# youmi-zym/GO-SLAM

Hardware: AMD Instinct MI355X
Metric: BA keyframes/s (6 x FactorGraph.update: reproject + corr lookup + GRU + 2 GN BA iters) on synthetic 640x480 RGB-D (higher is better)
Workload: dtype f32 (BA/geometry; fp64 solve), f16 (corr volume, GRU convs); 1 GPU; configs[1]-shaped frontend window: 60x80 maps (480x640 RGB-D), P=25 keyframes, E=75 edges, 6 updates/keyframe, iters=2, RGB-D depth prior, upsample on; parallelism=replicas x1 (tracking does not shard)

## Files before the change

go_slam_amd/_lib.py:

```python
import ctypes
import os
import subprocess

_HERE = os.path.dirname(os.path.abspath(__file__))
CSRC = os.path.join(_HERE, "csrc")
LIB_PATH = os.environ.get("GOSLAM_HIP_LIB") or os.path.join(CSRC, "libgoslam_hip.so")

_lib = None

c_int, c_float, c_void_p, c_size_t = ctypes.c_int, ctypes.c_float, ctypes.c_void_p, ctypes.c_size_t

_P = c_void_p
SIGNATURES = {
    "gs_version": (ctypes.c_char_p, []),
    "gs_last_error": (ctypes.c_char_p, []),
    "gs_enc_conv_wpack_elems": (c_size_t, [c_int, c_int, c_int]),
    "gs_enc_conv_stat_chunks": (c_int, [c_int, c_int, c_int]),
    "gs_enc_conv": (c_int, [_P, c_int, c_int, _P, _P, _P, c_int, c_int, c_int, c_int, c_int, c_int, c_int, _P, _P, _P]),
    "gs_norm_act_workspace_bytes_chunks": (c_size_t, [c_int, c_int, c_int]),
    "gs_timing_begin": (c_int, [_P]),
    "gs_timing_end": (c_int, []),
    "gs_timing_read": (c_int, [ctypes.c_char_p, ctypes.POINTER(ctypes.c_double), ctypes.POINTER(c_int)]),
    "gs_timing_names": (c_int, [ctypes.c_char_p, c_int]),
    "gs_corr_index_forward": (c_int, [_P, _P, _P] + [c_int] * 7 + [_P]),
# ... 11 lines not shown
    "gs_altcorr_pyramid": (c_int, [_P] * 8 + [c_int] * 5 + [_P]),
    "gs_reproject": (c_int, [_P] * 7 + [c_int] * 3 + [_P]),
    "gs_projmap": (c_int, [_P] * 7 + [c_int] * 3 + [_P]),
    "gs_frame_distance": (c_int, [_P] * 6 + [c_int] * 3 + [c_float, _P]),
    "gs_iproj": (c_int, [_P] * 4 + [c_int] * 3 + [_P]),
    "gs_depth_filter": (c_int, [_P] * 6 + [c_int] * 4 + [_P]),
    "gs_pointcloud_workspace_bytes": (c_size_t, [c_int] * 3),
    "gs_pointcloud_count": (c_int, [_P] * 5 + [c_float, c_float] + [c_int] * 4 + [_P, c_size_t, _P]),
    "gs_pointcloud_mask": (c_int, [_P, _P] + [c_int] * 4 + [_P, c_size_t, _P]),
    "gs_pointcloud_scan": (c_int, [c_int] * 3 + [_P, c_size_t, _P, _P]),
    "gs_pointcloud_emit": (c_int, [_P] * 5 + [c_int] * 4 + [_P, c_size_t, ctypes.c_longlong, _P, _P, _P]),
    "gs_tsdf_batch": (c_int, []),
    "gs_tsdf_integrate": (c_int, [_P] * 3 + [c_int] * 3 + [_P] * 4 + [c_int] * 3 + [c_float] * 10 + [_P]),
    "gs_tsdf_vertex_attr": (c_int, [_P, c_int, _P, _P, c_int, c_int, c_int, c_float, _P, _P, _P]),
    "gs_frame_prep_color": (c_int, [_P, c_int, c_int, c_int, c_int, c_int, _P]),
    "gs_frame_prep_depth": (c_int, [_P, c_int, c_float, c_int, c_int, c_int, c_int, _P]),
    "gs_cvx_upsample":(c_int, [_P] * 4 + [c_int] * 4 + [_P]),
    "gs_upmask_upsample": (c_int, [_P, c_int, _P, _P, _P, _P, _P, c_int, c_int, c_int, _P]),
    "gs_bias_act": (c_int, [_P, _P, _P, c_int, c_int, c_int, c_int, c_int, _P]),
    "gs_motion_features": (c_int, [_P, _P, _P, c_int, c_int, c_int, _P]),
    "gs_ba_inputs": (c_int, [_P] * 6 + [c_int, c_int, c_int, _P]),
    "gs_lowmem_gather": (c_int, [_P] * 7 + [c_int, c_int, c_int, _P]),
    "gs_lowmem_scatter": (c_int, [_P] * 8 + [c_int, c_int, c_int, _P]),
    "gs_damping_rows": (c_int, [_P] * 5 + [c_int, c_int, c_float, c_float, _P]),
    "gs_conv1x1": (c_int, [_P, c_int, c_int, _P, _P, c_int, _P, c_int, c_int, ctypes.c_longlong, _P]),
    "gs_conv7x7_c4": (c_int, [_P, _P, _P, _P, c_int, c_int, c_int, c_int, c_int, c_int, _P]),
    "gs_conv3x3_wpack_elems": (c_size_t, [c_int, c_int]),
    "gs_conv3x3_pp": (c_int, [_P, c_int, c_int, _P, c_int, _P, c_int, c_int, c_int, c_int, c_int, c_int, _P]),
    "gs_conv3x3_bias_relu": (c_int, [_P, c_int, c_int, _P, _P, _P, c_int, c_int, c_int, c_int, c_int, _P]),
    "gs_conv3x3_gru_zr": (c_int, [_P, c_int, c_int, _P, _P, _P, _P, _P, _P, c_int, c_int, c_int, _P]),
    "gs_conv3x3_gru_zr2": (c_int, [_P, _P, c_int, c_int, _P, _P, _P, _P, _P, _P, c_int, c_int, c_int, _P]),
    "gs_conv3x3_gru_q": (c_int, [_P, _P, c_int, c_int, _P, _P, _P, _P, _P, _P, _P, c_int, c_int, c_int, _P]),
    "gs_conv3x3_head": (c_int, [_P, c_int, _P, c_int, _P, _P, c_int, c_int, c_float, _P, c_int, c_int, c_int, _P]),
    "gs_segment_mean": (c_int, [_P, c_int, _P, c_int, _P, _P, _P, c_int, c_int, c_int, _P]),
    "gs_norm_act_workspace_bytes": (c_size_t, [c_int, c_int, c_int]),
    "gs_norm_act": (c_int, [_P, _P, _P, _P] + [c_int] * 6 + [c_float, _P, c_size_t, c_int, _P]),
    "gs_gru_glo_workspace_bytes": (c_size_t, [c_int]),
    "gs_gru_glo": (c_int, [_P] * 11 + [c_int, c_int, _P, c_size_t, _P]),
    "gs_gru_glo_fused_workspace_bytes": (c_size_t, [c_int, c_int]),
    "gs_gru_glo_fused": (c_int, [_P, c_int] + [_P] * 10 + [c_int, c_int, _P, c_size_t, _P]),
    "gs_gru_gate_zr": (c_int, [_P] * 6 + [c_int] * 3 + [_P]),
    "gs_gru_gate_q": (c_int, [_P] * 7 + [c_int] * 2 + [_P]),
    "gs_edge_prep": (c_int, [_P] * 4 + [c_int, _P, _P] + [c_int] * 6 + [c_float, c_int, c_int, _P]),
    "gs_edge_greedy": (c_int, [_P] * 5 + [c_int] * 5 + [c_float, c_int, c_int, _P]),
    "gs_ba_workspace_bytes": (c_size_t, [c_int] * 5),
    "gs_ba": (c_int, [_P] * 9 + [c_int] * 3 + [c_float, c_float] + [c_int] * 6 + [_P, _P, _P, _P, c_size_t, _P]),
    "gs_ba_ex": (c_int, [_P] * 9 + [c_int] * 3 + [c_float, c_float] + [c_int] * 6 + [_P, _P, _P, _P, c_size_t, c_int, _P]),
    "gs_chol_solve": (c_int, [_P, _P, c_int, c_float, c_float, c_int, _P, _P, _P]),
    "gs_traj_eval_workspace_bytes": (c_size_t, [c_int]),
    "gs_traj_world": (c_int, [_P, _P, c_int, _P, _P, _P]),
    "gs_ape_moments": (c_int, [_P, _P, _P, c_int, _P, _P, c_size_t, _P]),
    "gs_ape_stats": (c_int, [_P, _P, _P, _P, c_int, _P, _P, _P, c_size_t, _P]),
    "gs_grid_meta_default": (c_int, [_P]),
    "gs_neus_level_major_min_points": (c_int, [c_int]),
    "gs_render_sample": (c_int, [_P] * 7 + [c_float, _P, _P, _P] + [c_int] * 3 + [_P]),
    "gs_grid_encode": (c_int, [_P] * 4 + [c_int, _P]),
    "gs_grid_backward": (c_int, [_P, _P, _P, c_int, c_float, _P, _P, c_int, c_float, _P, _P, c_int, _P]),
    "gs_mlp_workspace_bytes": (c_size_t, [c_int, c_int]),
    "gs_mlp_forward": (c_int, [_P] * 3 + [c_int] * 3 + [_P, c_size_t, _P]),
    "gs_neus_forward_workspace_bytes": (c_size_t, [c_int, c_int]),
    "gs_neus_forward": (c_int, [_P] * 9 + [c_float] + [_P] * 18 + [c_float, _P, c_float, c_int, c_int, _P, c_size_t, _P]),
    "gs_neus_forward_pieces": (c_int, [c_int] * 3),
    "gs_neus_forward_segmented": (c_int, [_P] * 9 + [c_float] + [_P] * 18 + [c_float, c_int, _P, _P, c_float]
                                  + [c_int] * 4 + [_P, c_size_t, _P]),
    "gs_render_img_sample": (c_int, [_P, c_int, c_int] + [c_float] * 4 + [_P] * 5 + [c_int] + [_P] * 5
                             + [c_int, c_int, _P]),
# ... 155 lines not shown
```

go_slam_amd/csrc/conv3x3_pp.hip:

```cpp
#include "common.h"
#include "conv3x3_common.h"

namespace {

constexpr int PP_KG = 4;
constexpr int PP_PSTR = 5;
constexpr int pp_zpad(int tw) { return (((2 * (tw + 2) + 2) * PP_PSTR + 3 + 15) / 16) * 16; }
constexpr int pp_patch_slots(int tw) {
  return (((512 / tw + 2) * (tw + 2) * PP_PSTR + 511) / 512) * 512 + pp_zpad(tw);
}

__device__ __attribute__((aligned(16))) const uint32_t pp_zero_page[4] = {0u, 0u, 0u, 0u};

__device__ __forceinline__ void pp_glds16(const void* src, void* lds_wave_base) {
  __builtin_amdgcn_global_load_lds((const __attribute__((address_space(1))) void*)src,
                                   (__attribute__((address_space(3))) void*)lds_wave_base, 16, 0, 0);
}

#define PP_BAR()                              \
  do {                                        \
    asm volatile("" ::: "memory");            \
    __builtin_amdgcn_s_barrier();             \
    asm volatile("" ::: "memory");            \
    __builtin_amdgcn_sched_barrier(0);        \
  } while (0)

#define PP_LGKM0()                                        \
  do {                                                    \
    asm volatile("s_waitcnt lgkmcnt(0)" ::: "memory");    \
    __builtin_amdgcn_sched_barrier(0);                    \
  } while (0)

struct PpEpi {
  const float* bias;
  const float* glo;
  const _Float16* inp_pre;
  const _Float16* aux0;
  const _Float16* aux1;
  _Float16* out0;
  _Float16* out1;
  const _Float16* xb;
  int xsb, split;
  long long* dbg;
  int variant;
};

template <bool PROBE>
__device__ __forceinline__ void pp_stamp(long long* dbg, int slot) {
  if constexpr (PROBE) {
    if (dbg && threadIdx.x == 0) dbg[(size_t)blockIdx.x * 4 + slot] = (long long)__builtin_amdgcn_s_memtime();
  }
}

__device__ __forceinline__ float pp_sigm(float v) { return gs_sigmoid(v); }

template <int TW, int EPI, int BN = 128, bool PROBE = false>
__global__ __launch_bounds__(512, 1) void conv3x3_pp_kernel(const _Float16* __restrict__ x, int xs, int C,
                                                            const half8* __restrict__ wpack, _Float16* __restrict__ y,
                                                            int ys, int H, int W, int rows, int tiles_x, int NB,
                                                            int xcd, PpEpi ep) {
  static_assert(BN == 128 || (BN == 64 && (EPI == 0 || EPI == 3)), "64-channel workgroups: plain / bias + ReLU only");
  constexpr int PP_BN = BN;
  constexpr int PP_WTAP = PP_KG * PP_BN;
  constexpr int NJ = BN / 64;
  constexpr int PP_TS = NJ == 2 ? 72 : 40;
  constexpr int TH_ = 512 / TW, PW_ = TW + 2, NPX = (TH_ + 2) * PW_;
  constexpr int PSTR = PP_PSTR;
  constexpr int ZPAD = pp_zpad(TW);
  constexpr int NROUND = (NPX * PSTR + 511) / 512;
  constexpr int PSLOTS = NROUND * 512 + ZPAD;
  constexpr int ZSLOT = NROUND * 512;
  static_assert(PSLOTS == pp_patch_slots(TW), "launch_pp sizes the LDS with the same formula");
  static_assert(NROUND <= 9, "one DMA round per tap");
  extern __shared__ half8 smem[];
  half8* const pbuf = smem;
// ... 144 lines not shown
  for (int ck = 0; ck < nchunk; ++ck) {
#pragma unroll
    for (int tap = 0; tap < 9; ++tap) {
      const int tg = ck * 9 + tap;
      __builtin_amdgcn_sched_barrier(0);
      math([&]() {
        if constexpr (PROBE) {
          if (ep.variant & 4) return;
        }
        const int tw = tg + 3 < T ? tg + 3 : T - 1;
        issue_w(tw, (tg + 3) & 3);
        if (tap < NROUND) issue_patch(ck + 1 < nchunk ? ck + 1 : nchunk - 1, (ck + 1) & 1, tap, poff[tap]);
      });
      __builtin_amdgcn_sched_barrier(0);
      if (tap < NROUND) asm volatile("s_waitcnt vmcnt(2)" ::: "memory");
      else asm volatile("s_waitcnt vmcnt(1)" ::: "memory");
      PP_BAR();
      bool reads = true;
      if constexpr (PROBE) reads = !(ep.variant & 8);
      if (reads) {
        if (tap < 8) read_frags(ck & 1, (tg + 1) & 3, tap + 1);
        else if (ck + 1 < nchunk) read_frags((ck + 1) & 1, (tg + 1) & 3, 0);
      }
      PP_LGKM0();
      PP_BAR();
    }
  }
  pp_stamp<PROBE>(ep.dbg, 2);
  if (grp2 == 0) PP_BAR();
  asm volatile("s_waitcnt vmcnt(0)" ::: "memory");
  PP_BAR();

  _Float16* tile = reinterpret_cast<_Float16*>(smem) + wv * 32 * PP_TS;
  _Float16* yb = y + nb * PP_BN + wn * (PP_BN / 2);
  constexpr int PIECES = NJ * 4;
  constexpr int PXIT = 64 / PIECES;
  constexpr int NIT = 32 / PXIT;
#pragma unroll
  for (int i = 0; i < 4; ++i) {
    size_t pix4[NIT];
    bool ok4[NIT];
    half8 pi4[NIT], u4[NIT], v4[NIT];
    const int piece = lane & (PIECES - 1);
    const int c8 = wn * (PP_BN / 2) + piece * 8;
#pragma unroll
    for (int it = 0; it < NIT; ++it) {
      const int pxr = it * PXIT + lane / PIECES;
      int ty, tx;
      tile_pixel<TW, true>(wm, i, pxr, ty, tx);
      const int gv = g0 + ty, gx = tx0 + tx;
      ok4[it] = gv < rows && gx < W;
      pix4[it] = (size_t)gv * W + gx;
      if constexpr (EPI == 1 || EPI == 2) {
        const half8 z8 = {0, 0, 0, 0, 0, 0, 0, 0};
        pi4[it] = z8; u4[it] = z8; v4[it] = z8;
        if (ok4[it]) {
          if constexpr (EPI == 1) {
            if (ep.inp_pre) pi4[it] = *reinterpret_cast<const half8*>(ep.inp_pre + pix4[it] * 384 + nb * 128 + c8);
            if (nb == 1) u4[it] = *reinterpret_cast<const half8*>(x + pix4[it] * xs + c8);
          } else {
            if (ep.inp_pre) pi4[it] = *reinterpret_cast<const half8*>(ep.inp_pre + pix4[it] * 384 + 256 + c8);
            u4[it] = *reinterpret_cast<const half8*>(ep.aux0 + pix4[it] * 128 + c8);
            v4[it] = *reinterpret_cast<const half8*>(ep.aux1 + pix4[it] * 128 + c8);
          }
        }
      }
    }
#pragma unroll
    for (int j = 0; j < NJ; ++j)
#pragma unroll
      for (int g = 0; g < 4; ++g) {
        half4 o;
#pragma unroll
        for (int e = 0; e < 4; ++e) o[e] = (_Float16)acc[j][i][4 * g + e];
        *reinterpret_cast<half4*>(tile + r * PP_TS + j * 32 + 8 * g + 4 * kgl) = o;
      }
    __builtin_amdgcn_fence(__ATOMIC_RELEASE, "wavefront");
    __builtin_amdgcn_wave_barrier();
    __builtin_amdgcn_fence(__ATOMIC_ACQUIRE, "wavefront");
#pragma unroll
    for (int it = 0; it < NIT; ++it) {
      const int pxr = it * PXIT + lane / PIECES;
      if (ok4[it]) {
        const half8 v = *reinterpret_cast<const half8*>(tile + pxr * PP_TS + piece * 8);
        const size_t pix = pix4[it];
        if constexpr (EPI == 0) {
          *reinterpret_cast<half8*>(yb + pix * ys + piece * 8) = v;
        } else if constexpr (EPI == 3) {
          const float* bb = ep.bias + nb * PP_BN + c8;
          half8 o;
#pragma unroll
          for (int k = 0; k < 8; ++k) o[k] = (_Float16)fmaxf((float)v[k] + bb[k], 0.0f);
          *reinterpret_cast<half8*>(yb + pix * ys + piece * 8) = o;
        } else if constexpr (EPI == 1) {
          const int img = (int)(pix / ((size_t)H * W));
          const half8 pi = pi4[it];
          const float* bb = ep.bias + nb * 128 + c8;
          const float* gg = ep.glo + (size_t)img * 256 + nb * 128 + c8;
          half8 o;
          if (nb == 0) {
#pragma unroll
            for (int k = 0; k < 8; ++k) o[k] = (_Float16)pp_sigm((float)v[k] + (float)pi[k] + bb[k] + gg[k]);
            *reinterpret_cast<half8*>(ep.out0 + pix * 128 + c8) = o;
          } else {
            const half8 net = u4[it];
#pragma unroll
            for (int k = 0; k < 8; ++k)
              o[k] = (_Float16)(pp_sigm((float)v[k] + (float)pi[k] + bb[k] + gg[k]) * (float)net[k]);
            *reinterpret_cast<half8*>(ep.out1 + pix * 128 + c8) = o;
          }
        } else {
          const int img = (int)(pix / ((size_t)H * W));
          const half8 pi = pi4[it], zz = u4[it], nn = v4[it];
          const float* bb = ep.bias + c8;
          const float* gg = ep.glo + (size_t)img * 128 + c8;
          half8 o;
#pragma unroll
          for (int k = 0; k < 8; ++k) {
            const float a_ = (float)v[k] + (float)pi[k] + bb[k] + gg[k];
// ... 113 lines not shown
  if (n == 0) return GS_OK;
  PpEpi ep = PpEpi();
  ep.bias = bias_q;
  ep.glo = glo_q;
  ep.inp_pre = (const _Float16*)inp_pre;
  ep.aux0 = (const _Float16*)z;
  ep.aux1 = (const _Float16*)net;
  ep.out0 = (_Float16*)net_out;
  ep.xb = (const _Float16*)x_rest;
  ep.xsb = x_rest_stride;
  ep.split = 128;
  return dispatch_pp<2>(rnet, 128, 128 + c_rest, wpack, pp_tile_width(w), nullptr, 0, 128, n, h, w, 1,
                        (hipStream_t)stream, ep);
}

extern "C" int gs_conv3x3_bias_relu(const void* x, int x_stride, int c_in, const void* wpack, const float* bias, void* y,
                                    int y_stride, int n_out, int n, int h, int w, gs_stream_t stream) {
  GS_REQUIRE(x && wpack && bias && y, "conv3x3_bias_relu: null pointer");
  GS_REQUIRE(c_in > 0 && c_in % 32 == 0, "conv3x3_bias_relu: c_in must be a multiple of 32");
  GS_REQUIRE(n_out > 0 && n_out % 64 == 0, "conv3x3_bias_relu: n_out must be a multiple of 64");
  GS_REQUIRE(x_stride >= c_in && x_stride % 8 == 0, "conv3x3_bias_relu: bad x_stride");
  GS_REQUIRE(y_stride >= n_out && y_stride % 8 == 0, "conv3x3_bias_relu: bad y_stride");
  GS_REQUIRE(n >= 0 && h > 0 && w > 0, "conv3x3_bias_relu: bad shape");
  if (n == 0) return GS_OK;
  PpEpi ep = PpEpi();
  ep.bias = bias;
  if (pp_block_channels(n_out) == 64)
    return dispatch_pp<3, 64>(x, x_stride, c_in, wpack, pp_tile_width(w), y, y_stride, n_out, n, h, w, 1,
                              (hipStream_t)stream, ep);
  return dispatch_pp<3>(x, x_stride, c_in, wpack, pp_tile_width(w), y, y_stride, n_out, n, h, w, 1, (hipStream_t)stream,
                        ep);
}

extern "C" size_t gs_conv3x3_wpack_elems(int c_in, int n_out) { return (size_t)9 * c_in * n_out; }

#ifdef GS_BUILD_PROBES
extern "C" int gs_conv3x3_pp_probe(const void* x, int x_stride, int c_in, const void* wpack, int tw, void* y, int y_stride,
                                   int n_out, int n, int h, int w, int variant, long long* dbg, gs_stream_t stream) {
  GS_REQUIRE(x && wpack && y, "conv3x3_pp_probe: null pointer");
  GS_REQUIRE(tw == 16 && c_in > 0 && c_in % 32 == 0 && n_out > 0 && n_out % 128 == 0 && n > 0,
             "conv3x3_pp_probe: bad arguments (tw must be 16)");
  PpEpi ep = PpEpi();
  ep.dbg = dbg;
  ep.variant = variant;
  return launch_pp<16, 0, 128, true>(x, x_stride, c_in, wpack, y, y_stride, n_out, n, h, w, 1, (hipStream_t)stream, ep);
}
#endif
```

go_slam_amd/csrc/conv_heads.hip:

```cpp
#include "common.h"

namespace {

typedef _Float16 half8 __attribute__((ext_vector_type(8)));
typedef float float16v __attribute__((ext_vector_type(16)));

constexpr int HEAD_ROWS = 6;

template <int O>
__global__ __launch_bounds__(256) void conv3x3_head_kernel(
    const _Float16* __restrict__ x, int ldx, const float* __restrict__ in_bias, int in_relu,
    const _Float16* __restrict__ wpack, const float* __restrict__ bias, int epilogue, float out_scale,
    float* __restrict__ out, int h, int w) {
  constexpr int NT = 9 * O;
  constexpr int S = NT | 1;
  extern __shared__ float cs[];
  const int n = blockIdx.y;
  const int r0 = blockIdx.x * HEAD_ROWS;
  const int in_lo = max(r0 - 1, 0), in_hi = min(r0 + HEAD_ROWS, h - 1);
  const int npx = (in_hi - in_lo + 1) * w;
  const int tid = threadIdx.x, lane = tid & 63, wv = tid >> 6;
  const int kh = 8 * (lane >> 5);

  half8 a[8];
// ... 57 lines not shown
  }
  __syncthreads();

  const int nrow = min(HEAD_ROWS, h - r0);
  for (int idx = tid; idx < nrow * w; idx += 256) {
    const int r = r0 + idx / w, cc = idx % w;
    float acc[O];
#pragma unroll
    for (int o = 0; o < O; ++o) acc[o] = 0.0f;
#pragma unroll
    for (int ky = 0; ky < 3; ++ky) {
      const int rr = r + ky - 1;
      if (rr < 0 || rr >= h) continue;
#pragma unroll
      for (int kx = 0; kx < 3; ++kx) {
        const int c2 = cc + kx - 1;
        if (c2 < 0 || c2 >= w) continue;
        const float* p = cs + ((rr - in_lo) * w + c2) * S + (ky * 3 + kx) * O;
#pragma unroll
        for (int o = 0; o < O; ++o) acc[o] += p[o];
      }
    }
    float* op = out + ((size_t)(n * h + r) * w + cc) * O;
#pragma unroll
    for (int o = 0; o < O; ++o) {
      float v = (float)(_Float16)(acc[o] + bias[o]);
      if (epilogue == 1) v = (float)(_Float16)gs_sigmoid(v);
      else if (epilogue == 2) v = (v > 20.0f) ? v : log1pf(__expf(v));
      op[o] = v * out_scale;
    }
  }
}

template <int O>
int launch_head(const void* x, int ldx, const float* in_bias, int in_relu, const void* wpack, const float* bias,
                int epilogue, float out_scale, float* out, int n, int h, int w, hipStream_t st) {
  constexpr int S = (9 * O) | 1;
  const size_t lds = (size_t)(HEAD_ROWS + 2) * w * S * sizeof(float);
  GS_REQUIRE(lds <= 160 * 1024 - 512, "conv3x3_head: image width %d needs %zu bytes of LDS", w, lds);
  static GsLdsLimit limit;
  if (int rc = limit.raise((const void*)conv3x3_head_kernel<O>, lds, "conv3x3_head")) return rc;
  conv3x3_head_kernel<O><<<dim3(gs_cdiv(h, HEAD_ROWS), n), 256, lds, st>>>(
      (const _Float16*)x, ldx, in_bias, in_relu, (const _Float16*)wpack, bias, epilogue, out_scale, out, h, w);
  GS_CHECK_LAUNCH("conv3x3_head");
  return GS_OK;
}

}

extern "C" int gs_conv3x3_head(const void* x, int x_stride, const float* in_bias, int in_relu, const void* wpack,
                               const float* bias, int n_out, int epilogue, float out_scale, float* out, int n,
                               int h, int w, gs_stream_t stream) {
  GS_REQUIRE(x && wpack && bias && out, "conv3x3_head: null pointer");
  GS_REQUIRE(x_stride >= 128 && x_stride % 8 == 0, "conv3x3_head: x_stride must be >= 128 and a multiple of 8");
  GS_REQUIRE(n_out == 1 || n_out == 2, "conv3x3_head: n_out must be 1 or 2");
  GS_REQUIRE(epilogue >= 0 && epilogue <= 2, "conv3x3_head: epilogue in {0 none, 1 sigmoid, 2 softplus}");
  GS_REQUIRE(n >= 0 && h > 0 && w > 0, "conv3x3_head: bad shape");
  if (n == 0) return GS_OK;
  hipStream_t st = (hipStream_t)stream;
  return n_out == 1 ? launch_head<1>(x, x_stride, in_bias, in_relu, wpack, bias, epilogue, out_scale, out, n, h, w, st)
                    : launch_head<2>(x, x_stride, in_bias, in_relu, wpack, bias, epilogue, out_scale, out, n, h, w, st);
}
```

go_slam_amd/droid_net.py:

```python
import os

import torch
import torch.nn as nn
import torch.nn.functional as F

from .weight_packs import WeightPacks, conv_pack, tensors_key


class GradientClip(nn.Module):

    def forward(self, x):
        return x


def segment_mean(x, index, num_segments):
    n = x.shape[0]
    onehot = torch.zeros(num_segments, n, dtype=x.dtype, device=x.device)
    onehot[index, torch.arange(n, device=x.device)] = 1
    cnt = onehot.sum(dim=1, keepdim=True).clamp(min=1)
    avg = (onehot / cnt)
    if x.is_contiguous(memory_format=torch.channels_last):
        flat = x.permute(0, 2, 3, 1).reshape(n, -1)
        out = (avg @ flat).view(num_segments, x.shape[2], x.shape[3], x.shape[1])
        return out.permute(0, 3, 1, 2)
# ... 66 lines not shown

def conv7x7_c4_supported(conv, x):
    return (x.is_cuda and x.dtype == torch.float16 and x.dim() == 4 and x.shape[1] == 4 and x.shape[3] <= 1024
            and tuple(conv.weight.shape) == (128, 4, 7, 7) and conv.stride in (1, (1, 1))
            and conv.padding in (3, (3, 3)) and x.is_contiguous(memory_format=torch.channels_last))


def conv7x7_c4_bias_act(cache, conv, x, act, rt=0):
    from . import _lib
    wpack, bias = conv_pack(cache, conv, "7x7", pack_conv7x7_c4_weight)
    n, _, h, w = x.shape
    y = torch.empty((n, 128, h, w), dtype=torch.float16, device=x.device, memory_format=torch.channels_last)
    with torch.cuda.device(x.device):
        rc = _lib.lib().gs_conv7x7_c4(_lib.ptr(x), _lib.ptr(wpack), _lib.ptr(bias), _lib.ptr(y), 128, n, h, w,
                                      int(act == "relu"), int(rt), _lib.stream_ptr(x.device))
    _lib.check(rc, "conv7x7_c4")
    return y


def conv3x3_head(x, conv, cache, epilogue="none", out_scale=1.0, in_channel=0, in_bias=None, in_relu=False):
    from . import _lib
    wpack, bias = conv_pack(cache, conv, "head", pack_head_weight)
    n, C, h, w = x.shape
    O = conv.weight.shape[0]
    out = torch.empty(n, h, w, O, dtype=torch.float32, device=x.device)
    epi = {"none": 0, "sigmoid": 1, "softplus": 2}[epilogue]
    rc = _lib.lib().gs_conv3x3_head(x.data_ptr() + 2 * in_channel, C, _lib.ptr(in_bias), int(in_relu),
                                    _lib.ptr(wpack), _lib.ptr(bias), O, epi, float(out_scale), _lib.ptr(out),
                                    n, h, w, _lib.stream_ptr(x.device))
    _lib.check(rc, "conv3x3_head")
    return out


def cvx_upsample(data, mask):
    b, h, w, d = data.shape
    data = data.permute(0, 3, 1, 2)
    wts = torch.softmax(mask.view(b, 1, 9, 8, 8, h, w), dim=2)
    nb = F.unfold(data, kernel_size=3, padding=1).view(b, d, 9, 1, 1, h, w)
    up = (wts * nb).sum(dim=2)
    return up.permute(0, 4, 2, 5, 3, 1).reshape(b, 8 * h, 8 * w, d)


_HalfWeights = WeightPacks
_ACT = {"none": 0, "relu": 1, "sigmoid": 2}


def bias_act(y, b, act, out=None, out_channel=0, in_channel=0, channels=None):
    from . import _lib
    n, cy, h, wd = y.shape
    c = cy - in_channel if channels is None else channels
    dst, ldy, off = (y, cy, in_channel) if out is None else (out, out.shape[1], out_channel)
    rc = _lib.lib().gs_bias_act(y.data_ptr() + 2 * in_channel, _lib.ptr(b), dst.data_ptr() + 2 * off, n * h * wd, c,
                                cy, ldy, _ACT[act], _lib.stream_ptr(y.device))
    _lib.check(rc, "bias_act")
    return dst


CONV3X3_IMPL = "own"
GRU_FUSED_EPILOGUE = True
CONV7X7_OWN = True
GRU_GLO_FUSED = True
FUSE_UPMASK_UPSAMPLE = True
FUSE_LOOKUP_ENCODER = True
_CONV3X3_PACKS = {}
_CONV3X3_PACKS_MAX = 32


def pack_conv3x3_weight(weight, kc=32):
    O, C, kh, kw = weight.shape
    bn = 128 if O % 128 == 0 else 64
    assert (kh, kw) == (3, 3) and O % bn == 0 and C % kc == 0 and kc == 32
    w = weight.detach().half().reshape(O // bn, bn, C // kc, kc // 8, 8, 3, 3)
    return w.permute(0, 2, 5, 6, 3, 1, 4).contiguous().reshape(-1)


def conv3x3_hip_supported(x, w):
    return (x.is_cuda and x.dtype == torch.float16 and x.dim() == 4 and tuple(w.shape[2:]) == (3, 3)
            and w.shape[0] % 64 == 0 and w.shape[1] % 32 == 0 and x.shape[1] == w.shape[1]
            and x.is_contiguous(memory_format=torch.channels_last))


def _use_own_conv3x3(x, w, stride, padding):
    if CONV3X3_IMPL == "miopen" or stride not in (1, (1, 1)) or padding not in (1, (1, 1)):
        return False
    return conv3x3_hip_supported(x, w)


def conv3x3_weight_image(w, kc):
    key = (w.data_ptr(), w._version, tuple(w.shape), w.device, kc)
    hit = _CONV3X3_PACKS.pop(key, None)
    if hit is None:
        hit = (pack_conv3x3_weight(w, kc), w)
        while len(_CONV3X3_PACKS) >= _CONV3X3_PACKS_MAX:
            _CONV3X3_PACKS.pop(next(iter(_CONV3X3_PACKS)))
    _CONV3X3_PACKS[key] = hit
# ... 330 lines not shown
            inp_pre = self.gru.inp_gates(inp4)
        except torch.OutOfMemoryError:
            cache.clear()
            torch.cuda.empty_cache()
            inp_pre = self.gru.inp_gates(inp4)
        for k in [k for k, e in cache.items() if e[2] != wkey or e[0]() is None]:
            del cache[k]

        def _gone(_ref, key=key, cache_ref=weakref.ref(cache)):
            c = cache_ref()
            if c is not None:
                e = c.get(key)
                if e is not None and e[0] is _ref:
                    del c[key]
        cache[key] = (weakref.ref(owner, _gone), inp._version, wkey, inp_pre,
                      self._checksum(inp) if self.cache_check else None)
        nbytes = lambda e: sum(x.numel() * x.element_size()
                               for x in (e[3] if isinstance(e[3], (tuple, list)) else (e[3],)) if torch.is_tensor(x))
        total = sum(nbytes(e) for e in cache.values())
        cap = self._cache_cap(inp.device)
        while (total > cap or len(cache) > self.INP_CACHE_ENTRIES) and len(cache) > 1:
            _, e = cache.popitem(last=False)
            total -= nbytes(e)
        return hx, inp_pre

    def _head_weights(self):
        mods = (self.delta[0], self.weight[0], self.agg.conv1)

        def build():
            w = torch.cat([m.weight for m in mods], 0).detach().half().contiguous(memory_format=torch.channels_last)
            return w, [m.bias.detach().float().contiguous() for m in mods]
        return self._packs.get("heads", [m.weight for m in mods] + [m.bias for m in mods], build)

    def _corr_independent_part(self, net4, inp, f4, n, ht, wd):
        hx, inp_pre = self._edge_state(inp, n, ht, wd)
        if CONV7X7_OWN and conv7x7_c4_supported(self.flow_encoder[0], f4):
            f4 = conv7x7_c4_bias_act(self._packs, self.flow_encoder[0], f4, "relu")
        else:
            f4 = conv_bias_act(self._packs, self.flow_encoder[0], f4, "relu")
        conv_bias_act(self._packs, self.flow_encoder[2], f4, "relu", out=hx, out_channel=256)
        with torch.autocast("cuda", enabled=False):
            glo = self.gru.global_context(net4)
        return hx, inp_pre, glo

    def _forward_fast(self, net, inp, corr, flow, ii, jj, seg=None):
        batch, num, ch, ht, wd = net.shape
        cl = torch.channels_last
        packs = self._packs
        out_dim = (batch, num, -1, ht, wd)
        n = batch * num
        net4 = net.view(n, -1, ht, wd)
        from .corr import LazyLookup
        lazy = corr if isinstance(corr, LazyLookup) and FUSE_LOOKUP_ENCODER and corr.block.fused_encoder_supported() \
            else None
        if lazy is None:
            if isinstance(corr, LazyLookup):
                corr = corr.materialize()
            c4 = corr.view(n, -1, ht, wd).half().contiguous(memory_format=cl)
        if flow is None:
            flow = torch.zeros(batch, num, 4, ht, wd, device=net.device)
        f4 = flow.view(n, -1, ht, wd).half().contiguous(memory_format=cl)
        hx, inp_pre, glo = self._corr_independent_part(net4, inp, f4, n, ht, wd)
        if lazy is not None:
            c4 = lazy.encoded(*self._corr_enc0_padded())
        else:
            c4 = conv1x1_bias_act(packs, self.corr_encoder[0], c4, "relu")
        conv_bias_act(packs, self.corr_encoder[2], c4, "relu", out=hx, out_channel=128)
        net4 = self.gru.forward_hx(net4, hx, inp_pre, glo=glo)
        net = net4.view(*out_dim)
        hw_, hb = self._head_weights()
        heads = conv_nobias(net4, hw_ if ii is not None else hw_[:256], padding=1)
        delta = conv3x3_head(heads, self.delta[2], packs, "none", in_channel=0, in_bias=hb[0], in_relu=True)
        weight = conv3x3_head(heads, self.weight[2], packs, "sigmoid", in_channel=128, in_bias=hb[1], in_relu=True)
        delta, weight = delta.view(batch, num, ht, wd, 2), weight.view(batch, num, ht, wd, 2)
        if ii is None:
            return net, delta, weight
        agg = self.agg
        if seg is None:
            seg = build_segments(ii.to(net.device))
        x = segment_mean_hip(heads, seg, in_channel=256, channels=128, in_bias=hb[2], in_relu=True)
        x = conv_bias_act(packs, agg.conv2, x, "relu")
        eta = conv3x3_head(x, agg.eta[0], packs, "softplus", out_scale=0.01).view(batch, -1, ht, wd)
        if FUSE_UPMASK_UPSAMPLE:
            upmask = LazyUpmask(self, x, (batch, -1, 8 * 8 * 9, ht, wd))
        else:
            upmask = conv1x1_bias_act(packs, agg.upmask[0], x, "none").view(batch, -1, 8 * 8 * 9, ht, wd)
        return net, delta, weight, eta, upmask

    def _corr_enc0_padded(self):
        def pad(weight):
            w = torch.zeros(128, 208, dtype=torch.float16, device=weight.device)
            w[:, :196] = weight.detach().reshape(128, 196).half()
            return w
        return conv_pack(self._packs, self.corr_encoder[0], "pad208", pad)

    def _fast_ok(self, net, inp, corr):
        cl = torch.channels_last
        n4 = net.view(-1, *net.shape[2:])
        return (self.fuse_epilogues and net.is_cuda and not torch.is_grad_enabled() and net.dtype == torch.float16
                and net.shape[2] == 128 and n4.is_contiguous(memory_format=cl) and torch.is_autocast_enabled())

    def forward(self, net, inp, corr, flow=None, ii=None, jj=None, seg=None):
        batch, num, ch, ht, wd = net.shape
        if self._fast_ok(net, inp, corr):
            return self._forward_fast(net, inp, corr, flow, ii, jj, seg)
        if hasattr(corr, "materialize"):
            corr = corr.materialize()
        if flow is None:
            flow = torch.zeros(batch, num, 4, ht, wd, device=net.device)
        out_dim = (batch, num, -1, ht, wd)
        net = net.view(batch * num, -1, ht, wd)
        inp = inp.view(batch * num, -1, ht, wd)
        corr = self.corr_encoder(corr.view(batch * num, -1, ht, wd))
# ... 30 lines not shown
```

include/goslam_hip.h:

```cpp
#ifndef GOSLAM_HIP_H
#define GOSLAM_HIP_H

#include <stddef.h>
#include <stdint.h>

#ifdef __cplusplus
extern "C" {
#endif

typedef void* gs_stream_t;

typedef enum {
  GS_OK = 0,
  GS_ERR_INVALID_ARG = -1,
  GS_ERR_WORKSPACE = -2,
  GS_ERR_LAUNCH = -3,
  GS_ERR_UNSUPPORTED = -4
} gs_status;

typedef enum { GS_F16 = 0, GS_F32 = 1, GS_F64 = 2 } gs_dtype;

const char* gs_version(void);
const char* gs_last_error(void);

// ... 116 lines not shown
int gs_bias_act(const void* x, const float* bias, void* y, int rows, int channels, int x_stride, int y_stride,
                int act, gs_stream_t stream);
int gs_motion_features(const float* coords1, const float* target, void* out, int n, int h, int w,
                       gs_stream_t stream);
int gs_lowmem_gather(const float* coords1, const float* target, const void* net, const int64_t* sel,
                     float* coords_out, void* motion_out, void* net_out, int n_sel, int h, int w, gs_stream_t stream);
int gs_lowmem_scatter(const float* coords, const float* delta, const float* weight, const void* net_new,
                      const int64_t* sel, float* target, float* weight_all, void* net, int n_sel, int h, int w,
                      gs_stream_t stream);

int gs_ba_inputs(const float* coords1, const float* delta, const float* weight, float* target,
                 float* ba_target, float* ba_weight, int n, int h, int w, gs_stream_t stream);
int gs_conv1x1(const void* x, int x_stride, int k_in, const void* wpack, const float* bias, int act, void* y,
               int y_stride, int n_out, long long rows, gs_stream_t stream);
int gs_conv7x7_c4(const void* x, const void* wpack, const float* bias, void* y, int ys, int n, int h, int w, int relu,
                  int rt, gs_stream_t stream);
size_t gs_conv3x3_wpack_elems(int c_in, int n_out);
int gs_conv3x3_pp(const void* x, int x_stride, int c_in, const void* wpack, int tw, void* y, int y_stride, int n_out,
                  int n, int h, int w, int xcd_order, gs_stream_t stream);
int gs_conv3x3_bias_relu(const void* x, int x_stride, int c_in, const void* wpack, const float* bias, void* y,
                         int y_stride, int n_out, int n, int h, int w, gs_stream_t stream);
int gs_conv3x3_gru_zr2(const void* net, const void* x_rest, int x_rest_stride, int c_rest, const void* wpack,
                       const float* bias_zr, const float* glo_zr, const void* inp_pre, void* z_out, void* rnet_out,
                       int n, int h, int w, gs_stream_t stream);
int gs_conv3x3_gru_zr(const void* hx, int hx_stride, int c_in, const void* wpack, const float* bias_zr,
                      const float* glo_zr, const void* inp_pre, void* z_out, void* rnet_out, int n, int h, int w,
                      gs_stream_t stream);
int gs_conv3x3_gru_q(const void* rnet, const void* x_rest, int x_rest_stride, int c_rest, const void* wpack,
                     const float* bias_q, const float* glo_q, const void* inp_pre, const void* z, const void* net,
                     void* net_out, int n, int h, int w, gs_stream_t stream);
int gs_conv3x3_head(const void* x, int x_stride, const float* in_bias, int in_relu, const void* wpack,
                    const float* bias, int n_out, int epilogue, float out_scale, float* out, int n, int h, int w,
                    gs_stream_t stream);
int gs_segment_mean(const void* x, int x_stride, const float* in_bias, int in_relu, const int* seg_offsets,
                    const int* seg_edges, void* out, int n_seg, int hw, int channels, gs_stream_t stream);
size_t gs_norm_act_workspace_bytes(int n, int hw, int channels);
size_t gs_norm_act_workspace_bytes_chunks(int n, int chunks, int channels);
size_t gs_enc_conv_wpack_elems(int ksize, int c_in, int c_out);
int gs_enc_conv_stat_chunks(int h_out, int w_out, int c_out);
int gs_enc_conv(const void* x, int x_stride, int c_in, const void* wpack, const void* bias, void* y, int y_stride,
                int c_out, int ksize, int stride, int n, int h, int w, const void* stat_bias, void* stats_ws,
                gs_stream_t stream);
int gs_norm_act(const void* x, const void* bias, const void* skip, void* y, int n, int hw, int channels,
                int instance_norm, int relu_in, int relu_out, float eps, void* workspace, size_t workspace_bytes,
                int stat_chunks, gs_stream_t stream);
size_t gs_gru_glo_workspace_bytes(int n);
int gs_gru_glo(const void* w_pre, const float* w_bias, const void* net, const void* wz, const void* wr,
               const void* wq, const float* bz, const float* br, const float* bq, float* gzr, float* gq,
               int n, int hw, void* workspace, size_t workspace_bytes, gs_stream_t stream);

size_t gs_gru_glo_fused_workspace_bytes(int n, int hw);
int gs_gru_glo_fused(const void* net, int net_stride, const void* w_pack, const float* w_bias, const void* wz,
                     const void* wr, const void* wq, const float* bz, const float* br, const float* bq, float* gzr,
                     float* gq, int n, int hw, void* workspace, size_t workspace_bytes, gs_stream_t stream);

int gs_damping_rows(const float* eta, const int* inv, const int64_t* index, float* damping_buf, float* out,
                    int n_rows, int hw, float scale, float eps, gs_stream_t stream);

int gs_cvx_upsample(const float* disps, const void* mask, const int64_t* ix, float* out,
                    int m, int h, int w, int mask_channels_last, gs_stream_t stream);
int gs_upmask_upsample(const void* x, int x_stride, const void* weight, const float* bias, const float* disps,
                       const int64_t* ix, float* out, int m, int h, int w, gs_stream_t stream);


size_t gs_ba_workspace_bytes(int n_edges, int n_poses, int n_depth, int nbuf, int hw);

// ... 38 lines not shown
```

Before: 81.01 keyframes/s.

## Fuse head tap projection into conv3x3 epilogue with separate finish kernel

After: 83.00 keyframes/s (median of 6 runs). +2.4%, better.

```diff
diff --git a/go_slam_amd/_lib.py b/go_slam_amd/_lib.py
--- a/go_slam_amd/_lib.py
+++ b/go_slam_amd/_lib.py
@@ -67,6 +67,8 @@
     "gs_conv3x3_gru_zr2": (c_int, [_P, _P, c_int, c_int, _P, _P, _P, _P, _P, _P, c_int, c_int, c_int, _P]),
     "gs_conv3x3_gru_q": (c_int, [_P, _P, c_int, c_int, _P, _P, _P, _P, _P, _P, _P, c_int, c_int, c_int, _P]),
     "gs_conv3x3_head": (c_int, [_P, c_int, _P, c_int, _P, _P, c_int, c_int, c_float, _P, c_int, c_int, c_int, _P]),
+    "gs_conv3x3_heads": (c_int, [_P, c_int, c_int, _P, c_int, _P, _P, c_int, _P, _P, c_int, c_int, c_int, c_int, c_int, _P]),
+    "gs_conv3x3_heads_finish": (c_int, [_P, _P, _P, c_int, c_int, c_float, c_float, _P, _P, c_int, c_int, c_int, _P]),
     "gs_segment_mean": (c_int, [_P, c_int, _P, c_int, _P, _P, _P, c_int, c_int, c_int, _P]),
     "gs_norm_act_workspace_bytes": (c_size_t, [c_int, c_int, c_int]),
     "gs_norm_act": (c_int, [_P, _P, _P, _P] + [c_int] * 6 + [c_float, _P, c_size_t, c_int, _P]),
diff --git a/go_slam_amd/csrc/conv3x3_pp.hip b/go_slam_amd/csrc/conv3x3_pp.hip
--- a/go_slam_amd/csrc/conv3x3_pp.hip
+++ b/go_slam_amd/csrc/conv3x3_pp.hip
@@ -41,6 +41,9 @@
   _Float16* out1;
   const _Float16* xb;
   int xsb, split;
+  const half8* tapw;
+  float* tap_out;
+  int n_tap;
   long long* dbg;
   int variant;
 };
@@ -251,7 +254,89 @@
   PP_BAR();
 
   _Float16* tile = reinterpret_cast<_Float16*>(smem) + wv * 32 * PP_TS;
-  _Float16* yb = y + nb * PP_BN + wn * (PP_BN / 2);
+  _Float16* yb = y + (EPI == 4 ? nb - ep.n_tap : nb) * PP_BN + wn * (PP_BN / 2);
+  if constexpr (EPI == 4) {
+    if (nb < ep.n_tap) {
+      typedef float float4v __attribute__((ext_vector_type(4)));
+      typedef float float2v __attribute__((ext_vector_type(2)));
+      float4v* const hand = reinterpret_cast<float4v*>(reinterpret_cast<_Float16*>(smem) + 8 * 32 * PP_TS);
+      static_assert((8 * 32 * PP_TS * 2) % 16 == 0 && 8 * 32 * PP_TS * 2 + 2 * 4 * 4096 <= 2 * PSLOTS * 16, "hand-over");
+      half8 ta[4];
+      float tb[4][8];
+#pragma unroll
+      for (int ks = 0; ks < 4; ++ks) {
+        ta[ks] = ep.tapw[((size_t)nb * 8 + wn * 4 + ks) * 64 + lane];
+        const float* bb = ep.bias + nb * 128 + wn * 64 + 16 * ks + 8 * kgl;
+#pragma unroll
+        for (int e = 0; e < 8; ++e) tb[ks][e] = bb[e];
+      }
+      float* const tp = ep.tap_out + (size_t)nb * ((size_t)rows * W) * 18;
+#pragma unroll
+      for (int i = 0; i < 4; ++i) {
+#pragma unroll
+        for (int j = 0; j < NJ; ++j)
+#pragma unroll
+          for (int g = 0; g < 4; ++g) {
+            half4 o;
+#pragma unroll
+            for (int e = 0; e < 4; ++e) o[e] = (_Float16)acc[j][i][4 * g + e];
+            *reinterpret_cast<half4*>(tile + r * PP_TS + j * 32 + 8 * g + 4 * kgl) = o;
+          }
+        __builtin_amdgcn_fence(__ATOMIC_RELEASE, "wavefront");
+        __builtin_amdgcn_wave_barrier();
+        __builtin_amdgcn_fence(__ATOMIC_ACQUIRE, "wavefront");
+        half8 t[4];
+#pragma unroll
+        for (int ks = 0; ks < 4; ++ks) {
+          t[ks] = *reinterpret_cast<const half8*>(tile + r * PP_TS + 16 * ks + 8 * kgl);
+#pragma unroll
+          for (int e = 0; e < 8; ++e) {
+            float f = (float)t[ks][e] + tb[ks][e];
+            f = fmaxf(f, 0.0f);
+            t[ks][e] = (_Float16)f;
+          }
+        }
+        float4v* const hp = hand + (((i & 1) * 4 + wm) * 4) * 64 + lane;
+        float16v c;
+        if (wn == 0) {
+#pragma unroll
+          for (int e = 0; e < 16; ++e) c[e] = 0.0f;
+#pragma unroll
+          for (int ks = 0; ks < 4; ++ks) c = __builtin_amdgcn_mfma_f32_32x32x16_f16(ta[ks], t[ks], c, 0, 0, 0);
+#pragma unroll
+          for (int q = 0; q < 4; ++q) {
+            const float4v v = {c[4 * q], c[4 * q + 1], c[4 * q + 2], c[4 * q + 3]};
+            hp[q * 64] = v;
+          }
+        }
+        __syncthreads();
+        if (wn == 1) {
+#pragma unroll
+          for (int q = 0; q < 4; ++q) {
+            const float4v v = hp[q * 64];
+#pragma unroll
+            for (int e = 0; e < 4; ++e) c[4 * q + e] = v[e];
+          }
+#pragma unroll
+          for (int ks = 0; ks < 4; ++ks) c = __builtin_amdgcn_mfma_f32_32x32x16_f16(ta[ks], t[ks], c, 0, 0, 0);
+          int ty, tx;
+          tile_pixel<TW, true>(wm, i, r, ty, tx);
+          const int gv = g0 + ty, gx = tx0 + tx;
+          if (gv < rows && gx < W) {
+            float* o = tp + ((size_t)gv * W + gx) * 18 + 4 * kgl;
+            *reinterpret_cast<float2v*>(o) = float2v{c[0], c[1]};
+            *reinterpret_cast<float2v*>(o + 2) = float2v{c[2], c[3]};
+            *reinterpret_cast<float2v*>(o + 8) = float2v{c[4], c[5]};
+            *reinterpret_cast<float2v*>(o + 10) = float2v{c[6], c[7]};
+            if (kgl == 0) *reinterpret_cast<float2v*>(o + 16) = float2v{c[8], c[9]};
+          }
+        }
+        __builtin_amdgcn_fence(__ATOMIC_RELEASE, "wavefront");
+        __builtin_amdgcn_wave_barrier();
+      }
+      return;
+    }
+  }
   constexpr int PIECES = NJ * 4;
   constexpr int PXIT = 64 / PIECES;
   constexpr int NIT = 32 / PXIT;
@@ -303,7 +388,7 @@
       if (ok4[it]) {
         const half8 v = *reinterpret_cast<const half8*>(tile + pxr * PP_TS + piece * 8);
         const size_t pix = pix4[it];
-        if constexpr (EPI == 0) {
+        if constexpr (EPI == 0 || EPI == 4) {
           *reinterpret_cast<half8*>(yb + pix * ys + piece * 8) = v;
         } else if constexpr (EPI == 3) {
           const float* bb = ep.bias + nb * PP_BN + c8;
@@ -483,6 +568,28 @@
                         ep);
 }
 
+extern "C" int gs_conv3x3_heads(const void* x, int x_stride, int c_in, const void* wpack, int tw, const void* tap_wpack,
+                                const float* in_bias, int n_tap_blocks, float* tap_out, void* y, int y_stride, int n_out,
+                                int n, int h, int w, gs_stream_t stream) {
+  GS_REQUIRE(x && wpack && tap_wpack && in_bias && tap_out, "conv3x3_heads: null pointer");
+  GS_REQUIRE(tw == 8 || tw == 16, "conv3x3_heads: tile width must be 8 or 16");
+  GS_REQUIRE(c_in > 0 && c_in % 32 == 0, "conv3x3_heads: c_in must be a multiple of 32");
+  GS_REQUIRE(n_out > 0 && n_out % 128 == 0, "conv3x3_heads: n_out must be a multiple of 128");
+  GS_REQUIRE(n_tap_blocks >= 1 && n_tap_blocks <= n_out / 128, "conv3x3_heads: n_tap_blocks must be in [1, n_out / 128]");
+  GS_REQUIRE(x_stride >= c_in && x_stride % 8 == 0, "conv3x3_heads: x_stride must be >= c_in and a multiple of 8");
+  const int rest = n_out - 128 * n_tap_blocks;
+  GS_REQUIRE(rest == 0 || (y && y_stride >= rest && y_stride % 8 == 0),
+             "conv3x3_heads: y / y_stride must hold the %d channels behind the tap blocks", rest);
+  GS_REQUIRE(n >= 0 && h > 0 && w > 0, "conv3x3_heads: bad shape");
+  if (n == 0) return GS_OK;
+  PpEpi ep = PpEpi();
+  ep.bias = in_bias;
+  ep.tapw = (const half8*)tap_wpack;
+  ep.tap_out = tap_out;
+  ep.n_tap = n_tap_blocks;
+  return dispatch_pp<4>(x, x_stride, c_in, wpack, tw, y, y_stride, n_out, n, h, w, 1, (hipStream_t)stream, ep);
+}
+
 extern "C" size_t gs_conv3x3_wpack_elems(int c_in, int n_out) { return (size_t)9 * c_in * n_out; }
 
 #ifdef GS_BUILD_PROBES
diff --git a/go_slam_amd/csrc/conv_heads.hip b/go_slam_amd/csrc/conv_heads.hip
--- a/go_slam_amd/csrc/conv_heads.hip
+++ b/go_slam_amd/csrc/conv_heads.hip
@@ -113,6 +113,66 @@
   }
 }
 
+struct HeadsFinish {
+  const float* bias[2];
+  float* out[2];
+  int epilogue[2];
+  float scale[2];
+};
+
+__global__ __launch_bounds__(256) void conv3x3_heads_finish_kernel(const float* __restrict__ T, HeadsFinish p, int h, int w) {
+  constexpr int O = 2, NT = 9 * O, S = NT | 1;
+  typedef float float2v __attribute__((ext_vector_type(2)));
+  extern __shared__ float cs[];
+  const int n = blockIdx.y, hd = blockIdx.z;
+  const int r0 = blockIdx.x * HEAD_ROWS;
+  const int in_lo = max(r0 - 1, 0), in_hi = min(r0 + HEAD_ROWS, h - 1);
+  const int npx = (in_hi - in_lo + 1) * w;
+  const int tid = threadIdx.x;
+  const size_t npix = (size_t)gridDim.y * h * w;
+  const float2v* src = reinterpret_cast<const float2v*>(T + ((size_t)hd * npix + (size_t)(n * h + in_lo) * w) * NT);
+  for (int i = tid; i < npx * (NT / 2); i += 256) {
+    const float2v v = src[i];
+    const int px = i / (NT / 2), c = 2 * (i - (NT / 2) * px);
+    cs[px * S + c] = v[0];
+    cs[px * S + c + 1] = v[1];
+  }
+  __syncthreads();
+
+  const float* bias = p.bias[hd];
+  const int epilogue = p.epilogue[hd];
+  const float out_scale = p.scale[hd];
+  float* out = p.out[hd];
+  const int nrow = min(HEAD_ROWS, h - r0);
+  for (int idx = tid; idx < nrow * w; idx += 256) {
+    const int r = r0 + idx / w, cc = idx % w;
+    float acc[O];
+#pragma unroll
+    for (int o = 0; o < O; ++o) acc[o] = 0.0f;
+#pragma unroll
+    for (int ky = 0; ky < 3; ++ky) {
+      const int rr = r + ky - 1;
+      if (rr < 0 || rr >= h) continue;
+#pragma unroll
+      for (int kx = 0; kx < 3; ++kx) {
+        const int c2 = cc + kx - 1;
+        if (c2 < 0 || c2 >= w) continue;
+        const float* q = cs + ((rr - in_lo) * w + c2) * S + (ky * 3 + kx) * O;
+#pragma unroll
+        for (int o = 0; o < O; ++o) acc[o] += q[o];
+      }
+    }
+    float* op = out + ((size_t)(n * h + r) * w + cc) * O;
+#pragma unroll
+    for (int o = 0; o < O; ++o) {
+      float v = (float)(_Float16)(acc[o] + bias[o]);
+      if (epilogue == 1) v = (float)(_Float16)gs_sigmoid(v);
+      else if (epilogue == 2) v = (v > 20.0f) ? v : log1pf(__expf(v));
+      op[o] = v * out_scale;
+    }
+  }
+}
+
 template <int O>
 int launch_head(const void* x, int ldx, const float* in_bias, int in_relu, const void* wpack, const float* bias,
                 int epilogue, float out_scale, float* out, int n, int h, int w, hipStream_t st) {
@@ -142,3 +202,28 @@
   return n_out == 1 ? launch_head<1>(x, x_stride, in_bias, in_relu, wpack, bias, epilogue, out_scale, out, n, h, w, st)
                     : launch_head<2>(x, x_stride, in_bias, in_relu, wpack, bias, epilogue, out_scale, out, n, h, w, st);
 }
+
+extern "C" int gs_conv3x3_heads_finish(const float* tap, const float* bias0, const float* bias1, int epilogue0,
+                                       int epilogue1, float out_scale0, float out_scale1, float* out0, float* out1, int n,
+                                       int h, int w, gs_stream_t stream) {
+  GS_REQUIRE(tap && bias0 && bias1 && out0 && out1, "conv3x3_heads_finish: null pointer");
+  GS_REQUIRE(epilogue0 >= 0 && epilogue0 <= 2 && epilogue1 >= 0 && epilogue1 <= 2,
+             "conv3x3_heads_finish: epilogue in {0 none, 1 sigmoid, 2 softplus}");
+  GS_REQUIRE(n >= 0 && h > 0 && w > 0, "conv3x3_heads_finish: bad shape");
+  if (n == 0) return GS_OK;
+  const long long npix = (long long)n * h * w;
+  GS_REQUIRE(npix < (1ll << 29), "conv3x3_heads_finish: too many pixels");
+  HeadsFinish p;
+  p.bias[0] = bias0; p.bias[1] = bias1;
+  p.out[0] = out0; p.out[1] = out1;
+  p.epilogue[0] = epilogue0; p.epilogue[1] = epilogue1;
+  p.scale[0] = out_scale0; p.scale[1] = out_scale1;
+  GS_REQUIRE(n <= 65535, "conv3x3_heads_finish: at most 65535 images");
+  const size_t lds = (size_t)(HEAD_ROWS + 2) * w * 19 * sizeof(float);
+  GS_REQUIRE(lds <= 160 * 1024, "conv3x3_heads_finish: image width %d needs %zu bytes of LDS", w, lds);
+  static GsLdsLimit limit;
+  if (int rc = limit.raise((const void*)conv3x3_heads_finish_kernel, lds, "conv3x3_heads_finish")) return rc;
+  conv3x3_heads_finish_kernel<<<dim3(gs_cdiv(h, HEAD_ROWS), n, 2), 256, lds, (hipStream_t)stream>>>(tap, p, h, w);
+  GS_CHECK_LAUNCH("conv3x3_heads_finish");
+  return GS_OK;
+}
diff --git a/go_slam_amd/droid_net.py b/go_slam_amd/droid_net.py
--- a/go_slam_amd/droid_net.py
+++ b/go_slam_amd/droid_net.py
@@ -122,6 +122,37 @@
     return out
 
 
+def pack_heads_tap_weights(weights):
+    assert all(tuple(w.shape) == (2, 128, 3, 3) for w in weights)
+    return torch.stack([pack_head_weight(w) for w in weights]).contiguous()
+
+
+def heads_workspace_shapes(n, h, w, n_out, n_tap):
+    assert n_out % 128 == 0 and 1 <= n_tap <= n_out // 128
+    rest = n_out - 128 * n_tap
+    return (n_tap, n * h * w, 18), ((n, h, w, rest) if rest else None)
+
+
+def conv3x3_heads_fused(x, w, tap_wpack, in_bias, taps, rest, bias0, bias1, epilogues=("none", "sigmoid"), tw=None):
+    from . import _lib
+    image = conv3x3_weight_image(w, 32)
+    n, c, h, wd = x.shape
+    O = w.shape[0]
+    epi = {"none": 0, "sigmoid": 1, "softplus": 2}
+    out0 = torch.empty(n, h, wd, 2, dtype=torch.float32, device=x.device)
+    out1 = torch.empty(n, h, wd, 2, dtype=torch.float32, device=x.device)
+    L = _lib.lib()
+    with torch.cuda.device(x.device):
+        st = _lib.stream_ptr(x.device)
+        rc = L.gs_conv3x3_heads(_lib.ptr(x), c, c, _lib.ptr(image), tw or conv3x3_pp_tile_width(wd), _lib.ptr(tap_wpack),
+                                _lib.ptr(in_bias), 2, _lib.ptr(taps), _lib.ptr(rest), O - 256, O, n, h, wd, st)
+        _lib.check(rc, "conv3x3_heads")
+        rc = L.gs_conv3x3_heads_finish(_lib.ptr(taps), _lib.ptr(bias0), _lib.ptr(bias1), epi[epilogues[0]],
+                                       epi[epilogues[1]], 1.0, 1.0, _lib.ptr(out0), _lib.ptr(out1), n, h, wd, st)
+        _lib.check(rc, "conv3x3_heads_finish")
+    return out0, out1
+
+
 def cvx_upsample(data, mask):
     b, h, w, d = data.shape
     data = data.permute(0, 3, 1, 2)
@@ -151,6 +182,7 @@
 CONV7X7_OWN = True
 GRU_GLO_FUSED = True
 FUSE_UPMASK_UPSAMPLE = True
+FUSE_HEAD_TAPS = True
 FUSE_LOOKUP_ENCODER = True
 _CONV3X3_PACKS = {}
 _CONV3X3_PACKS_MAX = 32
@@ -547,6 +579,32 @@
             return w, [m.bias.detach().float().contiguous() for m in mods]
         return self._packs.get("heads", [m.weight for m in mods] + [m.bias for m in mods], build)
 
+    def _head_taps(self):
+        mods = (self.delta[0], self.weight[0], self.delta[2], self.weight[2])
+
+        def build():
+            return (pack_heads_tap_weights([self.delta[2].weight, self.weight[2].weight]),
+                    torch.cat([self.delta[0].bias, self.weight[0].bias]).detach().float().contiguous(),
+                    self.delta[2].bias.detach().float().contiguous(), self.weight[2].bias.detach().float().contiguous())
+        return self._packs.get("head_taps", [m.weight for m in mods] + [m.bias for m in mods], build)
+
+    HEADS_WS_ENTRIES = 4
+
+    def _heads_workspace(self, n, ht, wd, n_out, device):
+        ws = self.__dict__.setdefault("_heads_ws", {})
+        key = (n, ht, wd, n_out, device)
+        hit = ws.pop(key, None)
+        if hit is None:
+            ts, rs = heads_workspace_shapes(n, ht, wd, n_out, 2)
+            taps = torch.empty(ts, dtype=torch.float32, device=device)
+            rest = None if rs is None else torch.empty((n, rs[3], ht, wd), dtype=torch.float16, device=device,
+                                                       memory_format=torch.channels_last)
+            hit = (taps, rest)
+            while len(ws) >= self.HEADS_WS_ENTRIES:
+                ws.pop(next(iter(ws)))
+        ws[key] = hit
+        return hit
+
     def _corr_independent_part(self, net4, inp, f4, n, ht, wd):
         hx, inp_pre = self._edge_state(inp, n, ht, wd)
         if CONV7X7_OWN and conv7x7_c4_supported(self.flow_encoder[0], f4):
@@ -584,16 +642,25 @@
         net4 = self.gru.forward_hx(net4, hx, inp_pre, glo=glo)
         net = net4.view(*out_dim)
         hw_, hb = self._head_weights()
-        heads = conv_nobias(net4, hw_ if ii is not None else hw_[:256], padding=1)
-        delta = conv3x3_head(heads, self.delta[2], packs, "none", in_channel=0, in_bias=hb[0], in_relu=True)
-        weight = conv3x3_head(heads, self.weight[2], packs, "sigmoid", in_channel=128, in_bias=hb[1], in_relu=True)
+        hw_ = hw_ if ii is not None else hw_[:256]
+        fused = FUSE_HEAD_TAPS and _use_own_conv3x3(net4, hw_, 1, 1)
+        if fused:
+            tapw, tapb, b_delta, b_weight = self._head_taps()
+            taps, heads = self._heads_workspace(n, ht, wd, hw_.shape[0], net4.device)
+            delta, weight = conv3x3_heads_fused(net4, hw_, tapw, tapb, taps, heads, b_delta, b_weight)
+            agg_channel = 0
+        else:
+            heads = conv_nobias(net4, hw_, padding=1)
+            delta = conv3x3_head(heads, self.delta[2], packs, "none", in_channel=0, in_bias=hb[0], in_relu=True)
+            weight = conv3x3_head(heads, self.weight[2], packs, "sigmoid", in_channel=128, in_bias=hb[1], in_relu=True)
+            agg_channel = 256
         delta, weight = delta.view(batch, num, ht, wd, 2), weight.view(batch, num, ht, wd, 2)
         if ii is None:
             return net, delta, weight
         agg = self.agg
         if seg is None:
             seg = build_segments(ii.to(net.device))
-        x = segment_mean_hip(heads, seg, in_channel=256, channels=128, in_bias=hb[2], in_relu=True)
+        x = segment_mean_hip(heads, seg, in_channel=agg_channel, channels=128, in_bias=hb[2], in_relu=True)
         x = conv_bias_act(packs, agg.conv2, x, "relu")
         eta = conv3x3_head(x, agg.eta[0], packs, "softplus", out_scale=0.01).view(batch, -1, ht, wd)
         if FUSE_UPMASK_UPSAMPLE:
diff --git a/include/goslam_hip.h b/include/goslam_hip.h
--- a/include/goslam_hip.h
+++ b/include/goslam_hip.h
@@ -172,6 +172,12 @@
 int gs_conv3x3_head(const void* x, int x_stride, const float* in_bias, int in_relu, const void* wpack,
                     const float* bias, int n_out, int epilogue, float out_scale, float* out, int n, int h, int w,
                     gs_stream_t stream);
+int gs_conv3x3_heads(const void* x, int x_stride, int c_in, const void* wpack, int tw, const void* tap_wpack,
+                     const float* in_bias, int n_tap_blocks, float* tap_out, void* y, int y_stride, int n_out, int n,
+                     int h, int w, gs_stream_t stream);
+int gs_conv3x3_heads_finish(const float* tap, const float* bias0, const float* bias1, int epilogue0, int epilogue1,
+                            float out_scale0, float out_scale1, float* out0, float* out1, int n, int h, int w,
+                            gs_stream_t stream);
 int gs_segment_mean(const void* x, int x_stride, const float* in_bias, int in_relu, const int* seg_offsets,
                     const int* seg_edges, void* out, int n_seg, int hw, int channels, gs_stream_t stream);
 size_t gs_norm_act_workspace_bytes(int n, int hw, int channels);
```
